# PolyChord/PolyChordLite

Hardware: AMD Instinct MI355X
Metric: likelihood evals/sec, 20D Gaussian nlive=2000 (higher is better)
Workload: dtype f64; 1 GPU; configs[1]: 20-D Gaussian, nlive=2000, num_repeats=40, one full run per step; batch_chains=1000, parallelism=repeat-sharded x1, mode=one run at a time per GPU; R runs in step: roofline.in_step

## Files before the change

include/polychord_hip.h:

```cpp
#ifndef POLYCHORD_HIP_H
#define POLYCHORD_HIP_H
#include <stdbool.h>
#ifdef __cplusplus
extern "C" {
#endif


typedef double (*polychord_loglike_fn)(double *theta, int nDims, double *phi, int nDerived);
typedef void (*polychord_prior_fn)(double *cube, double *theta, int nDims);
typedef void (*polychord_dumper_fn)(int ndead, int nlive, int npars, double *live, double *dead,
                                    double *logweights, double logZ, double logZerr);

void polychord_c_interface(
    polychord_loglike_fn loglikelihood, polychord_prior_fn prior, polychord_dumper_fn dumper,
    int nlive, int num_repeats, int nprior, int nfail, bool do_clustering, int feedback,
    double precision_criterion, double logzero, int max_ndead, double boost_posterior,
    bool posteriors, bool equals, bool cluster_posteriors, bool write_resume, bool write_paramnames,
    bool read_resume, bool write_stats, bool write_live, bool write_dead, bool write_prior,
    bool maximise, double compression_factor, bool synchronous, int nDims, int nDerived,
    char *base_dir, char *file_root, int nGrade, double *grade_frac, int *grade_dims, int n_nlives,
    double *loglikes, int *nlives, int seed, int *comm);

void polychord_c_interface_ini(polychord_loglike_fn loglikelihood, void (*setup_loglikelihood)(void),
                               char *inifile, int *comm);
// ... 246 lines not shown
                        unsigned batch, int nchains, const double *seeds, const double *chol,
                        double contour, double *babies_out, double *nhats_out, int *nlike_out);
#define PCHIP_NO_SUCH_PATH 64
int  pchip_directions(const pchip_settings *s, const pchip_like *like, const pchip_prior *prior, unsigned batch, int nchains,
                      const double *seeds, const double *chol, int path, double *nhat_out, double *nhat_w_out,
                      double *nhat_Ms_out, double *ch_My_out, int *has_Ms, double *raw_out, int nrows, int nbases);
int  pchip_prior_transform(const pchip_prior *prior, int nDims, int n, const double *cube, double *theta, int device);
int  pchip_update_factors(const pchip_settings *s, int ncluster, int nlive, const double *live, const int *live_cluster,
                          int nph, const double *phantom, const double *ph_logL, const int *ph_cluster, const double *threshold,
                          const double *shift, int path, double *cov, double *chol, int *count, double *shift_out, int *chol_suspect);
typedef struct {
    int ncluster, nlive, nph;
    const double *live, *live_logL; const int *live_cluster;
    const double *phantom, *ph_logL; const int *ph_cluster;
} pchip_cluster_in;
typedef struct {
    int maxc, nsplit_cap, scratch_cap;
    int ncluster, nsplit, levels, scratch_n;
    int *live_cluster, *live_pos, *cl_list;
    int *cl_n, *imin_slot, *ph_count; unsigned *cl_uid;
    double *logLp, *lse_ref, *lse_sum, *logXp, *logZp, *logZXp, *logZp2, *logZpXp;
    double *XpXq;
    int *ph_cluster;
    unsigned *split_child, *split_parent; double *split_logfrac;
    double *init;
    double *scratch_Sm; int *scratch_knn, *scratch_lab;
} pchip_cluster_out;
int  pchip_cluster_update(const pchip_settings *s, int nsets, const pchip_cluster_in *in, pchip_cluster_out *out, int path);

int  pchip_park_pack(int nchains, int nDims, const int *need, const double *prop, int *rank, int *count, double *cube, int device);
int  pchip_park_pack_many(int nruns, const int *nchains, int nDims, const int *need, const double *prop, int *rank, int *counts, int *total,
                          double *cube, int device);

#ifdef __cplusplus
}
#endif
#endif
```

polychordlite_amd/_ctypes_api.py:

```python
import ctypes as C
import os

import numpy as np

_HERE = os.path.dirname(os.path.abspath(__file__))
LIB_PATH = os.environ.get("PCHIP_LIB") or os.path.join(_HERE, "libpolychord_hip.so")

LOGLIKE_FN = C.CFUNCTYPE(C.c_double, C.POINTER(C.c_double), C.c_int, C.POINTER(C.c_double), C.c_int)
PRIOR_FN = C.CFUNCTYPE(None, C.POINTER(C.c_double), C.POINTER(C.c_double), C.c_int)
DUMPER_FN = C.CFUNCTYPE(None, C.c_int, C.c_int, C.c_int, C.POINTER(C.c_double), C.POINTER(C.c_double),
                        C.POINTER(C.c_double), C.c_double, C.c_double)

LIKE_CALLBACK, LIKE_GAUSSIAN, LIKE_RASTRIGIN, LIKE_TWIN_GAUSSIAN, LIKE_CORR_GAUSSIAN, LIKE_SOURCE = range(6)
KERNEL_CLASSES = ("k_nhats", "k_slice", "k_consume", "k_apply", "k_clean", "k_covmats", "k_bases_side")
LIKE_KINDS = {"gaussian": LIKE_GAUSSIAN, "rastrigin": LIKE_RASTRIGIN, "twin_gaussian": LIKE_TWIN_GAUSSIAN,
              "corr_gaussian": LIKE_CORR_GAUSSIAN, "source": LIKE_SOURCE}


class Settings(C.Structure):
    _fields_ = [("nDims", C.c_int), ("nDerived", C.c_int), ("nlive", C.c_int), ("num_repeats", C.c_int),
                ("nprior", C.c_int), ("nfail", C.c_int), ("do_clustering", C.c_int),
                ("precision_criterion", C.c_double), ("logzero", C.c_double), ("max_ndead", C.c_int),
                ("boost_posterior", C.c_double), ("posteriors", C.c_int), ("equals", C.c_int),
                ("cluster_posteriors", C.c_int), ("compression_factor", C.c_double), ("n_nlives", C.c_int),
# ... 91 lines not shown
    pr = np.ascontiguousarray(prop, dtype=np.float64)
    out = np.zeros_like(pr) if cube is None else cube
    assert out.flags.c_contiguous and out.dtype == np.float64 and out.shape == pr.shape
    rank = np.empty(nd.size, dtype=np.int32)
    cnt = C.c_int(-1)
    ip = C.POINTER(C.c_int)
    lib.pchip_park_pack.argtypes = [C.c_int, C.c_int, ip, C.POINTER(C.c_double), ip, ip, C.POINTER(C.c_double), C.c_int]
    lib.pchip_park_pack.restype = C.c_int
    rc = lib.pchip_park_pack(pr.shape[0], pr.shape[1], nd.ctypes.data_as(ip), dptr(pr), rank.ctypes.data_as(ip), C.byref(cnt), dptr(out), device)
    if rc:
        raise RuntimeError(f"pchip_park_pack failed with code {rc}")
    return rank, cnt.value, out


def park_pack_many(nchains, need, prop, cube=None, device=-1):
    lib = load()
    nc = np.ascontiguousarray(nchains, dtype=np.int32)
    nd = np.ascontiguousarray(need, dtype=np.int32)
    pr = np.ascontiguousarray(prop, dtype=np.float64)
    out = np.zeros_like(pr) if cube is None else cube
    assert out.flags.c_contiguous and out.dtype == np.float64 and out.shape == pr.shape
    assert nc.ndim == 1 and pr.ndim == 2 and nd.size == pr.shape[0] == int(nc.sum())
    rank = np.empty(nd.size, dtype=np.int32)
    counts = np.full(nc.size, -1, dtype=np.int32)
    tot = C.c_int(-1)
    ip = C.POINTER(C.c_int)
    lib.pchip_park_pack_many.argtypes = [C.c_int, ip, C.c_int, ip, C.POINTER(C.c_double), ip, ip, ip, C.POINTER(C.c_double), C.c_int]
    lib.pchip_park_pack_many.restype = C.c_int
    rc = lib.pchip_park_pack_many(nc.size, nc.ctypes.data_as(ip), pr.shape[1], nd.ctypes.data_as(ip), dptr(pr), rank.ctypes.data_as(ip),
                                  counts.ctypes.data_as(ip), C.byref(tot), dptr(out), device)
    if rc:
        raise RuntimeError(f"pchip_park_pack_many failed with code {rc}")
    return rank, counts, tot.value, out


_lib = None


def load():
    global _lib
    if _lib is not None:
        return _lib
    if not os.path.exists(LIB_PATH):
        raise ImportError(f"{LIB_PATH} is missing: build it with `python -m polychordlite_amd.build` "
                          "(hipcc --offload-arch=gfx950).  There is no CPU fallback.")
    lib = C.CDLL(LIB_PATH, mode=C.RTLD_GLOBAL)
    lib.pchip_settings_default.argtypes = [C.POINTER(Settings), C.c_int, C.c_int]
    lib.pchip_settings_default.restype = None
    lib.pchip_device_count.restype = C.c_int
    lib.pchip_run.argtypes = [C.POINTER(Settings), C.POINTER(Like), C.POINTER(Prior), C.POINTER(Result)]
    lib.pchip_run.restype = C.c_int
    lib.pchip_result_free.argtypes = [C.POINTER(Result)]
    lib.pchip_result_free.restype = None
    lib.pchip_slice_chains.argtypes = [C.POINTER(Settings), C.POINTER(Like), C.POINTER(Prior), C.c_uint, C.c_int,
                                       C.POINTER(C.c_double), C.POINTER(C.c_double), C.c_double,
                                       C.POINTER(C.c_double), C.POINTER(C.c_double), C.POINTER(C.c_int)]
    lib.pchip_slice_chains.restype = C.c_int
    lib.pchip_directions.argtypes = [C.POINTER(Settings), C.POINTER(Like), C.POINTER(Prior), C.c_uint, C.c_int, C.POINTER(C.c_double),
                                     C.POINTER(C.c_double), C.c_int, C.POINTER(C.c_double), C.POINTER(C.c_double), C.POINTER(C.c_double),
                                     C.POINTER(C.c_double), C.POINTER(C.c_int), C.POINTER(C.c_double), C.c_int, C.c_int]
    lib.pchip_directions.restype = C.c_int
    lib.polychord_hip_set_gaussian.argtypes = [C.c_double, C.c_double]
    lib.polychord_hip_set_uniform_prior.argtypes = [C.c_int, C.POINTER(C.c_double), C.POINTER(C.c_double)]
    lib.polychord_hip_set_corr_gaussian.argtypes = [C.c_int, C.POINTER(C.c_double), C.POINTER(C.c_double), C.c_double]
    lib.polychord_hip_set_option.argtypes = [C.c_char_p, C.c_double]
    lib.polychord_hip_set_sub_clustering.argtypes = [C.c_int, C.POINTER(C.c_int)]
# ... 475 lines not shown
```

polychordlite_amd/csrc/pc_engine.hip:

```cpp
#include "pc_state.h"
#include "pc_resume.h"
#include "pc_prior_table.h"
#include "pc_launch.h"
#include "pc_plan.h"
#include <cstdio>
#include <cstdlib>
#include <cstring>
#include <cstdarg>
#include <cstdint>
#include <new>
#include <cmath>
#include <vector>
#include <memory>
#include <string>
#include <chrono>
#include <algorithm>
#include <map>
#include <unordered_map>
#include <atomic>
#include <mutex>
#include <thread>
#include <functional>
#include <exception>
#include <ucontext.h>
// ... 2252 lines not shown
}

int pchip_park_pack(int nchains, int nDims, const int *need, const double *prop, int *rank, int *count, double *cube, int device)
{
    if (nchains < 1 || nDims < 1 || !need || !prop || !rank || !count || !cube) { pc_abi_set_last_error("pchip_park_pack: nchains >= 1 flags and rows of nDims >= 1, and room for the ranks, the count and the rows"); return 1; }
    int ndev = 0;
    if (hipGetDeviceCount(&ndev) != hipSuccess || ndev == 0) { (void)hipGetLastError(); std::fprintf(stderr, "polychord_hip: no HIP device available -- this engine has no CPU path\n"); return 2; }
    if (hipSetDevice(device >= 0 ? device % ndev : 0) != hipSuccess) return 2;
    const size_t nb = sizeof(double) * (size_t)nchains * nDims, ni = sizeof(int) * (size_t)nchains;
    int *d_need = nullptr, *d_rank = nullptr, *d_count = nullptr, *h_count = nullptr; double *d_prop = nullptr, *d_cube = nullptr;
    int rc = 2;
    if (hipMalloc(&d_need, ni) == hipSuccess && hipMalloc(&d_rank, ni) == hipSuccess && hipMalloc(&d_count, sizeof(int)) == hipSuccess &&
        hipMalloc(&d_prop, nb) == hipSuccess && hipMalloc(&d_cube, nb) == hipSuccess && hipHostMalloc(&h_count, sizeof(int)) == hipSuccess &&
        hipMemcpy(d_need, need, ni, hipMemcpyHostToDevice) == hipSuccess && hipMemcpy(d_prop, prop, nb, hipMemcpyHostToDevice) == hipSuccess &&
        hipMemcpy(d_cube, cube, nb, hipMemcpyHostToDevice) == hipSuccess) {
        void *dp = nullptr;
        *h_count = -1;
        if (hipHostGetDevicePointer(&dp, h_count, 0) == hipSuccess) {
            pc_launch_park_pack(nchains, nDims, d_need, 1, d_prop, d_rank, d_count, (int *)dp, d_cube, nullptr);
            int dc = -2;
            if (hipDeviceSynchronize() == hipSuccess && hipMemcpy(rank, d_rank, ni, hipMemcpyDeviceToHost) == hipSuccess &&
                hipMemcpy(&dc, d_count, sizeof(int), hipMemcpyDeviceToHost) == hipSuccess && hipMemcpy(cube, d_cube, nb, hipMemcpyDeviceToHost) == hipSuccess) {
                *count = *(volatile int *)h_count;
                rc = dc == *count ? 0 : 2;
            }
        }
    }
    if (rc) (void)hipGetLastError();
    (void)hipFree(d_need); (void)hipFree(d_rank); (void)hipFree(d_count); (void)hipFree(d_prop); (void)hipFree(d_cube);
    if (h_count) (void)hipHostFree(h_count);
    return rc;
}

int pchip_park_pack_many(int nruns, const int *nchains, int nDims, const int *need, const double *prop, int *rank, int *counts, int *total,
                         double *cube, int device)
{
    if (nruns < 1 || nruns > PC_PARK_MAX_RUNS || nDims < 1 || !nchains || !need || !prop || !rank || !counts || !total || !cube) {
        pc_abi_set_last_error("pchip_park_pack_many: 1 <= nruns <= 64 runs of nchains[r] >= 1 flags and rows of nDims >= 1, and room for the ranks, the counts, the total and the rows");
        return 1;
    }
    size_t all = 0; int max_chains = 0;
    for (int r = 0; r < nruns; ++r) {
        if (nchains[r] < 1) { pc_abi_set_last_error("pchip_park_pack_many: every run has at least one chain"); return 1; }
        all += (size_t)nchains[r]; max_chains = std::max(max_chains, nchains[r]);
    }
    int ndev = 0;
    if (hipGetDeviceCount(&ndev) != hipSuccess || ndev == 0) { (void)hipGetLastError(); std::fprintf(stderr, "polychord_hip: no HIP device available -- this engine has no CPU path\n"); return 2; }
    if (hipSetDevice(device >= 0 ? device % ndev : 0) != hipSuccess) return 2;
    const size_t nb = sizeof(double) * all * nDims, ni = sizeof(int) * all;
    int *d_need = nullptr, *d_rank = nullptr, *d_count = nullptr, *h_count = nullptr; double *d_prop = nullptr, *d_cube = nullptr; PcParkRun *h_runs = nullptr;
    int rc = 2;
    if (hipMalloc(&d_need, ni) == hipSuccess && hipMalloc(&d_rank, ni) == hipSuccess && hipMalloc(&d_count, sizeof(int) * PC_PARK_MAX_RUNS) == hipSuccess &&
        hipMalloc(&d_prop, nb) == hipSuccess && hipMalloc(&d_cube, nb) == hipSuccess && hipHostMalloc(&h_count, sizeof(int) * (PC_PARK_MAX_RUNS + 1)) == hipSuccess &&
        hipHostMalloc(&h_runs, sizeof(PcParkRun) * PC_PARK_MAX_RUNS) == hipSuccess &&
        hipMemcpy(d_need, need, ni, hipMemcpyHostToDevice) == hipSuccess && hipMemcpy(d_prop, prop, nb, hipMemcpyHostToDevice) == hipSuccess &&
        hipMemcpy(d_cube, cube, nb, hipMemcpyHostToDevice) == hipSuccess) {
        size_t o = 0;
        for (int r = 0; r < nruns; ++r) { h_runs[r] = PcParkRun{d_need + o, d_prop + o * nDims, d_rank + o, nchains[r], 1}; o += (size_t)nchains[r]; }
        for (int r = 0; r <= nruns; ++r) h_count[r] = -1;
        void *dp = nullptr, *dr = nullptr;
        if (hipHostGetDevicePointer(&dp, h_count, 0) == hipSuccess && hipHostGetDevicePointer(&dr, h_runs, 0) == hipSuccess &&
            pc_launch_park_pack_many(nruns, (const PcParkRun *)dr, max_chains, nDims, d_count, (int *)dp, d_cube, nullptr) == 0) {
            std::vector<int> dc((size_t)nruns, -2);
            if (hipDeviceSynchronize() == hipSuccess && hipMemcpy(rank, d_rank, ni, hipMemcpyDeviceToHost) == hipSuccess &&
                hipMemcpy(dc.data(), d_count, sizeof(int) * nruns, hipMemcpyDeviceToHost) == hipSuccess && hipMemcpy(cube, d_cube, nb, hipMemcpyDeviceToHost) == hipSuccess) {
                long sum = 0; rc = 0;
// ... 498 lines not shown
```

polychordlite_amd/csrc/pc_launch.h:

```cpp
#pragma once
#include "pc_state.h"
#include "../../include/polychord_hip.h"
#include <cstddef>
#include <memory>
#include <vector>

struct PcSourceForm {
    long nterms;
    int nsums;
    long nquad;
    long nshared;
    int has_prior;
    long long ndata, ntail;
    int alive;
};

static inline size_t pc_quad_lds(const PcSourceForm &f) { return f.nquad > 0 ? sizeof(double) * 2 * (size_t)((f.nquad + 1) & ~1L) : 0; }

static inline size_t pc_front_lds(const PcSourceForm &f) { return pc_quad_lds(f) + (f.nshared > 0 ? sizeof(double) * 2 * (size_t)((f.nshared + 1) & ~1L) : 0); }

static inline int pc_slice_phi_lds(const PcState *S, const PcSourceForm &f)
{
    const size_t sh0 = sizeof(double) * ((size_t)S->D + S->nr) + 16, tb = sizeof(double) * (size_t)S->nr * (S->D + 1);
    const size_t sums = sizeof(double) * (size_t)S->nr * (size_t)f.nsums;
// ... 40 lines not shown
int pc_launch_clean_many(const PcManyRec *dR, int R, int nblk_max, hipStream_t st);
void pc_launch_install_live(const PcState *S, const double *rows, int n, hipStream_t st);
void pc_launch_clean(const PcState *S, int nph, unsigned char *keep, int *blk, int *d_total, double *ph2, double *phL2, unsigned *phC2, unsigned long long *phU2, int *dst_index, hipStream_t st);
void pc_launch_reset_thresholds(const PcState *S, hipStream_t st);
int pc_launch_reset_thresholds_many(const PcState *S, const PcManyRec *dR, int R, hipStream_t st);
int pc_cov_nchunk(const PcState *S, int nph);
int pc_launch_covmats(const PcState *S, int nph, int nc, double *psum, int *pcnt, double *mean, int *count, double *pcov, hipStream_t st);
void pc_launch_scan_blocks(int *blk, int nblk, int *total, int *total2, hipStream_t st);
void pc_launch_chol_only(const PcState *S, const double *ncov, const int *count, hipStream_t st);
void pc_launch_init_state(const PcState *S, double logzero, hipStream_t st);
int pc_post_blocks(void);
void pc_launch_post_moments(const PcState *S, int nd, double *pmax, double *part, hipStream_t st);
void pc_prepare_streams(int dev, int want);
void *pc_cache_dev_alloc(size_t bytes);
void pc_cache_dev_free(void *p);
void *pc_cache_host_alloc(size_t bytes);
void pc_cache_host_free(void *p);
int pc_run_many(const pchip_settings *s, const pchip_like *like, const pchip_prior *prior, int nseeds, const int *seeds, int device, int max_in_flight, pchip_result *results);
void *pc_source_batch_open(int handle, int device, int nDims, int nDerived, polychord_prior_fn prior);
void pc_source_batch_eval(void *user, int n, int nDims, int nDerived, const double *cube, double *theta, double *phi, double *logL);
void pc_source_batch_close(void *user);
void pc_batch_callback_get(polychord_batch_fn *fn, void **user);
int pc_device_batch_registered(void);
int pc_fast_fits(const PcState *S);
int pc_launch_sort_live(const PcState *S, hipStream_t st);
int pc_launch_sort_live_many(const PcState *S, const PcManyRec *dR, int R, hipStream_t st);
int pc_launch_consume_fast(const PcState *S, int final_mode, hipStream_t st);
void pc_launch_ph_prepare(const PcState *S, hipStream_t st);
size_t pc_records_block_bytes(long long cap, int nT);
int pc_pack_lived_device(const double *dead, const double *logw, const double *entry, long long nd, int nT, double logzero, double *block, long long cap, long long *h_count, hipStream_t st);
int pc_par_fits(const PcState *S);
int pc_launch_consume_par(const PcState *S, hipStream_t st);
int pc_launch_consume_par_many(const PcState *S, const PcManyRec *dR, int R, hipStream_t st);
int pc_launch_final_par(const PcState *S, hipStream_t st);
int pc_launch_final_par_split(const PcState *S, hipStream_t st);
int pc_launch_final_par_many(const PcManyRec *dR, int R, hipStream_t st);
int pc_rtc_launch(const PcState *S, const char *expr, dim3 grid, dim3 block, size_t sh, hipStream_t st, void **args);
const char *pc_rtc_error(void);
int pc_rtc_source_form(int id, PcSourceForm *f);
int pc_rtc_wanted(const PcState *S);
int pc_launch_generate_live(const PcState *S, int attempt0, int n, double *rows, double *rows_logL, hipStream_t st);
int pc_nhats_splittable(const PcState *S);
int pc_launch_nhats_part(const PcState *S, unsigned batch, int nchains, int part, hipStream_t st, int packed);
int pc_launch_nhats(const PcState *S, unsigned batch, int nchains, hipStream_t st);
int pc_slice_fusable(const PcState *S);
int pc_launch_slice_fused(const PcState *S, unsigned batch, int nchains, hipStream_t st);
int pc_launch_slice_many(const PcState *S, const PcManyRec *dR, int R, int nchains, int fused, hipStream_t st);
int pc_launch_slice_step(const PcState *S, const PcManyRec *dR, int R, int nchains, int fused, hipStream_t st);
int pc_launch_nhats_many(const PcState *S, const PcManyRec *dR, int R, int nchains, hipStream_t st);
int pc_launch_slice(const PcState *S, unsigned batch, int nchains, hipStream_t st);
int pc_launch_prior_transform(const PcState *S, int n, const double *cubes, double *thetas, hipStream_t st);
int pc_launch_source_eval(const PcState *S, int n, const double *thetas, double *logL, double *phi, hipStream_t st);
int pc_launch_source_prior_eval(const PcState *S, int n, const double *cubes, double *thetas, hipStream_t st);
int pc_launch_max_rank(const PcState *S, int n, const double *rows, double *val, hipStream_t st);
int pc_launch_maximise(const PcState *S, int nprob, const double *in, const int *hdr, long long max_iter, double *out, long long *outi, hipStream_t st);
int pc_max_choose_simplex(int nDims, int nTotal, double logzero, const double *live, const int *cluster, int nlive, const double *vals,
                          double *simplex, double *f);
void pc_maximum_alloc(pchip_maximum *m, int nDims, int nDerived);
int pc_bases_t_ok(const PcState *S);
int pc_launch_bases_t(const PcState *S, unsigned batch, int nchains, hipStream_t st);
int pc_launch_bases_t_many(const PcState *S, const PcManyRec *dR, int R, unsigned batch, int nchains, hipStream_t st);
int pc_slice_t_ok(const PcState *S, int ncluster);
int pc_launch_slice_t(const PcState *S, unsigned batch, int nchains, hipStream_t st);
int pc_launch_slice_t_many(const PcState *S, const PcManyRec *dR, int R, unsigned batch, int nchains, hipStream_t st);
int pc_update_fused_ok(const PcState *S, int nc);
int pc_update_fused_blocks(const PcState *S, int nph);
// ... 13 lines not shown
```

polychordlite_amd/csrc/pc_par.hip:

```cpp
#include "pc_state.h"
#include "pc_launch.h"
#include "pc_keys.h"

typedef unsigned long long u64;
#define PAR_NT 1024
#define PAR_W 16

__device__ __forceinline__ int prefix_bits(const u64 *words, int t)
{
    int c = 0;
    const int wq = t >> 6;
    #pragma unroll
    for (int x = 0; x < PAR_W; ++x) {
        u64 v = words[x];
        if (x > wq) v = 0ull; else if (x == wq) v &= (1ull << (t & 63)) - 1ull;
        c += __popcll(v);
    }
    return c;
}

__device__ __forceinline__ int prefix_cum(const u64 *words, const int *cum, int t)
{
    const int wq = t >> 6;
    return (wq >= PAR_W) ? cum[PAR_W] : cum[wq] + __popcll(words[wq] & ((1ull << (t & 63)) - 1ull));
// ... 129 lines not shown
        R[q] = ref[q];
        const bool has = s[q] != 0.0 && m[q] > 0.5 * NEGBIG;
        const double d = m[q] - R[q];
        bad = bad || (has && !(fabs(d) <= PAR_LIN_SPAN));
        inc[q] = wave_scan_f64(has ? s[q] * exp(d) : 0.0, lane);
        if (lane == 63) sc[q * PAR_W + wv] = inc[q];
    }
    if (__ballot(bad) != 0ull && lane == 0) ref[NSEQ] = 1.0;
    pc_lds_barrier();
    const bool ok = ref[NSEQ] == 0.0;
    if (ok) {
        #pragma unroll
        for (int q = 0; q < NSEQ; ++q) {
            const double t = sc[q * PAR_W + (lane & 15)];
            double pre = t;
            pre += dpp_f64<0x111>(pre); pre += dpp_f64<0x112>(pre); pre += dpp_f64<0x114>(pre); pre += dpp_f64<0x118>(pre);
            s[q] = inc[q] + readlane_f64(pre - t, wv);
            m[q] = R[q];
        }
    }
    pc_lds_barrier();
    return ok;
}

__device__ __forceinline__ double block_scan_add(double v, int lane, int wv, double *wtot)
{
    v = wave_scan_f64(v, lane);
    if (lane == 63) wtot[wv] = v;
    __syncthreads();
    double p = 0.0;
    for (int x = 0; x < wv; ++x) p += wtot[x];
    __syncthreads();
    return v + p;
}

__device__ __forceinline__ void consume_par_body(const PcState &S)
{
    extern __shared__ __attribute__((aligned(16))) char smem[];
    const int tid = threadIdx.x, lane = tid & 63, wv = tid >> 6;
    const int Ncap = S.Ncap, nr = S.nr, NS = (Ncap + 63) & ~63;
    const int Bh = S.B;
    double bl = 0.0; int ep = 0, nl = 0;
    if (tid < Bh) { const int wh = Bh - 1 - tid; bl = S.baby_logL_T[(size_t)(nr - 1) * Bh + wh]; ep = S.ch_epoch[wh]; nl = S.ch_nlike[wh]; }
    PcCtl *ctl = S.ctl;
    const int T = ctl->i_nursery;
    const int n = S.cl_n[0];
    u64 *sSortK = (u64 *)smem;
    u64 *cK = sSortK + NS;
    u64 *srtK = cK + PAR_NT;
    u64 *uKey = srtK + PAR_NT;
    u64 *Gm = uKey + PAR_NT + 64;
    u64 *accR = Gm + PAR_NT;
    u64 *amask = accR + PAR_W;
    u64 *vmask = amask + PAR_W;
    double *sZi = (double *)(vmask + PAR_W);
    double *wtot = sZi + PAR_NT;
    double *fin = wtot + 64;
    int *sSort = (int *)(fin + 16);
    int *srtT = sSort + NS;
    int *rnk = srtT + PAR_NT;
    int *rlo = rnk + PAR_NT;
    int *uSrc = rlo + PAR_NT;
    int *slotA = uSrc + PAR_NT + 64;
    int *parA = slotA + PAR_NT;
    int *accStep = parA + PAR_NT;
    int *ish = accStep + PAR_NT;
    int *hist = ish + 16;
    double *X5 = (double *)(hist + NS + 64);
    double *sLse = (double *)Gm;

    const int epoch = ctl->admin_epoch;
    const int ndead0 = ctl->ndead, fail0 = ctl->failures, nph0 = ctl->nphantom;
    const long long nlike0 = ctl->nlike, niter0 = ctl->niter;
    const double logZ0 = ctl->logZ, logZ20 = ctl->logZ2;
    const double Xp0 = S.logXp[0], Zp0 = S.logZp[0], ZXp0 = S.logZXp[0], Zp20 = S.logZp2[0], ZpXp0 = S.logZpXp[0], XX0 = S.XpXq[0];
    const double lseRef0 = S.lse_ref[0], lseSum0 = S.lse_sum[0];
    const unsigned cuid = S.cl_uid[0];
    const double log2v = 0.6931471805599453;
    __shared__ int cumA[PAR_W + 1], cumV[PAR_W + 1], cumR[PAR_W + 1];
    __shared__ double ulog[4];
    if (wv == PAR_W - 1 && lane < 4) ulog[lane] = log(lane == 3 ? lseSum0 : (double)n + (double)lane);

    long long cyc[9]; int ncy = 0;
    cyc[ncy++] = clock64();
    for (int s = tid; s < Ncap; s += PAR_NT) { S.slot_src[s] = -1; if (S.defer_update) S.slot_step[s] = -1; }
    for (int i = tid; i < NS; i += PAR_NT) { sSortK[i] = (i < n) ? S.sort_key[i] : KEY_HUGE; sSort[i] = S.sort_slot[i]; }
    const bool inT = tid < T;
    const int w = T - 1 - tid;
    u64 ck = KEY_HUGE; bool valid = false;
    if (T != Bh && inT) { bl = S.baby_logL_T[(size_t)(nr - 1) * S.B + w]; ep = S.ch_epoch[w]; nl = S.ch_nlike[w]; }
    if (inT) { ck = d2key(bl); valid = ep == epoch; } else nl = 0;
    cK[tid] = ck;
    for (int i = tid; i < NS + 64; i += PAR_NT) hist[i] = 0;
    {
        const u64 vm = __ballot(valid);
        if (lane == 0) { vmask[wv] = vm; accR[wv] = 0ull; amask[wv] = 0ull; }
    }
    if (tid == 0) { ish[0] = (T << 2) | 3; ish[1] = 0; ish[3] = 0; }
    __syncthreads();
    const double l0 = ulog[0], l1 = ulog[1], l2 = ulog[2], d01 = l0 - l1, d02 = l0 - l2;

    int rl = 0, rp = 0;
    if (inT) {
        int lo = 0, hi = n;
        while (lo < hi) { const int mid = (lo + hi) >> 1; if (sSortK[mid] < ck) lo = mid + 1; else hi = mid; }
        rl = lo; rp = lo;
        while (rp < n && sSortK[rp] == ck) rp++;
    }
    rlo[tid] = rl;

    cyc[ncy++] = clock64();
    int myoff = 0;
    if (inT) myoff = atomicAdd(&hist[rl], 1);
    __syncthreads();
    {
        const int nb = n + 2;
        const int per = (nb + PAR_NT - 1) / PAR_NT, b0 = tid * per;
        int sum = 0;
        for (int x = 0; x < per; ++x) if (b0 + x < nb) sum += hist[b0 + x];
        int inc = sum;
        inc = wave_scan_i32(inc, lane);
        if (lane == 63) accStep[wv] = inc;
        __syncthreads();
        int run = inc - sum;
        for (int x = 0; x < wv; ++x) run += accStep[x];
        for (int x = 0; x < per; ++x) if (b0 + x < nb) { const int cnt = hist[b0 + x]; hist[b0 + x] = run; run += cnt; }
    }
    __syncthreads();
    if (inT) srtT[hist[rl] + myoff] = tid;
    __syncthreads();
    int rho = tid;
    if (inT) {
        const int g0 = hist[rl], g1 = hist[rl + 1];
        int below = 0;
        for (int x = g0; x < g1; ++x) {
            const int o = srtT[x];
            const u64 ko = cK[o];
            below += (ko < ck) || (ko == ck && o > tid);
        }
        rho = g0 + below;
    }
    rnk[tid] = rho;

    cyc[ncy++] = clock64();
    {
        u64 G = 0ull;
        #pragma unroll
        for (int j = 0; j < 64; ++j) {
            const int rj = __builtin_amdgcn_readlane(rho, j);
            if (j < lane && rj > rho) G |= 1ull << j;
        }
        Gm[tid] = G;
    }
    __syncthreads();
    if (wv == 0) {
        const int nch = (T + 63) >> 6;
        int *cum = accStep;
        if (lane < PAR_W) cum[lane] = 0;
        __threadfence_block();
        int rho_t = rnk[lane], r = rlo[lane], tot = 0;
        u64 Gt = Gm[lane];
        for (int c = 0; c < nch; ++c) {
            const int tn = (c + 1 < nch) ? (c + 1) * 64 + lane : lane;
            const int nrho = rnk[tn], nr2 = rlo[tn];
            const u64 nG = Gm[tn];
            const bool v = (vmask[c] >> lane) & 1ull;
            const int wq = rho_t >> 6, bq = rho_t & 63;
            const int P = tot - cum[wq] - __popcll(accR[wq] & (((1ull << bq) << 1) - 1ull));
            u64 am = __ballot(v && r > P);
            for (int it = 0; it < 66; ++it) {
                const bool a = v && r > P + __popcll(Gt & am);
                const u64 nm = __ballot(a);
                if (nm == am) break;
                am = nm;
            }
            if ((am >> lane) & 1ull) atomicOr(&accR[wq], 1ull << bq);
            if (lane == 0) amask[c] = am;
            tot += __popcll(am);
            PAR_WAVE_ORDER();
            {
                int cw = (lane < PAR_W) ? __popcll(accR[lane]) : 0, inc = cw;
                inc += dpp_i32<0x111>(inc); inc += dpp_i32<0x112>(inc); inc += dpp_i32<0x114>(inc); inc += dpp_i32<0x118>(inc);
                if (lane < PAR_W) cum[lane] = inc - cw;
            }
            PAR_WAVE_ORDER();
            rho_t = nrho; r = nr2; Gt = nG;
        }
        {
            const int ca = (lane < PAR_W) ? __popcll(amask[lane]) : 0, cv = (lane < PAR_W) ? __popcll(vmask[lane]) : 0,
                      cr = (lane < PAR_W) ? __popcll(accR[lane]) : 0;
            int ia = ca, iv = cv, ir = cr;
            ia += dpp_i32<0x111>(ia); ia += dpp_i32<0x112>(ia); ia += dpp_i32<0x114>(ia); ia += dpp_i32<0x118>(ia);
            iv += dpp_i32<0x111>(iv); iv += dpp_i32<0x112>(iv); iv += dpp_i32<0x114>(iv); iv += dpp_i32<0x118>(iv);
            ir += dpp_i32<0x111>(ir); ir += dpp_i32<0x112>(ir); ir += dpp_i32<0x114>(ir); ir += dpp_i32<0x118>(ir);
            if (lane < PAR_W) { cumA[lane] = ia - ca; cumV[lane] = iv - cv; cumR[lane] = ir - cr; }
            if (lane == PAR_W - 1) { cumA[PAR_W] = ia; cumV[PAR_W] = iv; cumR[PAR_W] = ir; }
        }
    }
    __syncthreads();

    cyc[ncy++] = clock64();
    const u64 amw = amask[wv], ltm = (1ull << lane) - 1ull;
    const bool acc = (amw >> lane) & 1ull;
    const int kt = cumA[wv] + __popcll(amw & ltm);
    const int K = cumA[PAR_W];
    const int vp = cumV[wv] + __popcll(vmask[wv] & ltm);
    int pos = 0, q = 0;
    if (acc) {
        q = cumR[rho >> 6] + __popcll(accR[rho >> 6] & ((1ull << (rho & 63)) - 1ull));
        pos = q + rp;
        accStep[kt] = tid; srtK[q] = ck;
    }
    __syncthreads();
    const u64 *aK = srtK;

    for (int idx = tid; idx <= K && idx < n; idx += PAR_NT) {
        const u64 sk = sSortK[idx];
        int lo = 0, hi = K;
        while (lo < hi) { const int mid = (lo + hi) >> 1; if (aK[mid] < sk) lo = mid + 1; else hi = mid; }
        const int p2 = idx + lo;
        if (p2 <= K) { uKey[p2] = sk; uSrc[p2] = sSort[idx]; }
    }
    if (acc && pos <= K) { uKey[pos] = ck; uSrc[pos] = -(1 + tid); }
    __syncthreads();

    const u64 gk = inT ? uKey[kt] : KEY_HUGE;
    const int src = acc ? uSrc[kt] : 0;
    slotA[tid] = (acc && src >= 0) ? src : -1;
    parA[tid] = (acc && src < 0) ? (-src - 1) : -1;
    __syncthreads();
    for (int it = 0; it < 12; ++it) {
        const int p = parA[tid];
// ... 254 lines not shown
            if (x > (ts >> 6)) word = 0ull; else if (x == (ts >> 6)) word &= (1ull << (ts & 63)) - 1ull;
            if (word) { tl = x * 64 + 63 - __clzll((long long)word); break; }
        }
        ctl->failures = (tl >= 0) ? vps - prefix_cum(vmask, cumV, tl) - 1 : fail0 + vps;
        ctl->status = status; ctl->error = (pri == 2) ? PC_ERR_DEAD_CAP : PC_ERR_NONE;
        ctl->i_nursery = T - ts; ctl->ndead = ndead0 + vps; ctl->seg_hi = T - 1; ctl->seg_lo = T - ts; ctl->cluster_deleted = 0;
        ctl->nlike = nlike0 + ish[1]; ctl->niter = niter0 + ts; ctl->nphantom = ish[2]; ctl->nlike_failed += ish[3];
        if (Kp) { ctl->logZ = fin[0]; ctl->logZ2 = fin[4]; }
        if (pri == 0) ctl->logX_last_update = Xp;
        ctl->upd_pending = 0; ctl->upd_marks = 0;
        if (marks_sh[1] > 0) {
            const int Kl = marks_sh[0], marks = marks_sh[1];
            ctl->upd_pending = 1; ctl->upd_marks = marks;
            ctl->upd_tmark = accStep[Kl - 1] + 1; ctl->upd_T = T; ctl->upd_ts = ts; ctl->upd_nph0 = S.pool ? S.pool_base : nph0;
            ctl->upd_thr = key2d(uKey[Kl - 1]); ctl->upd_keep_thr = (Kp > Kl) ? 1 : 0;
            ctl->logX_last_update = Xp0 + (double)Kl * d01;
        }
        if (S.use_prec) ctl->live_logZ = (Kp ? sLse[Kp - 1] : lseRef0 + ulog[3]) - l0 + Xp;
        cyc[ncy++] = clock64();
#ifdef PAR_NO_DBG
#elif defined(PAR_DBG_EVID)
        for (int x = 0; x < 7; ++x) ctl->dbg[x] += ecy[x + 1] - ecy[x];
#elif defined(PAR_DBG_PUBLISH)
        pcy[6] = clock64();
        for (int x = 0; x < 6; ++x) ctl->dbg[x] += pcy[x + 1] - pcy[x];
#else
        for (int x = 0; x + 1 < ncy && x < 8; ++x) ctl->dbg[x] += cyc[x + 1] - cyc[x];
        ctl->dbg[7] += npair;
#endif
    }
}
__global__ __launch_bounds__(PAR_NT) void k_consume_par(PcState S) { consume_par_body(S); }
__global__ __launch_bounds__(PAR_NT) void k_consume_par_many(const PcManyRec *R) { consume_par_body(pc_many_state(R, blockIdx.y)); }


template <bool ROWS>
__device__ __forceinline__ void final_par_body(const PcState &S)
{
    __shared__ __attribute__((aligned(16))) double X0[PAR_NT], X1[PAR_NT], X2[PAR_NT], X3[PAR_NT];
    __shared__ double wtot[64];
    __shared__ double carry[12];
    const int tid = threadIdx.x, lane = tid & 63, wv = tid >> 6;
    PcCtl *ctl = S.ctl;
    const int n0 = S.cl_n[0], nT = S.nT, ndead0 = ctl->ndead;
    const unsigned cuid = S.cl_uid[0];
    const double log2v = 0.6931471805599453;
    if (ndead0 + n0 > S.Dcap) { if (tid == 0) { ctl->status = PC_ST_ERROR; ctl->error = PC_ERR_DEAD_CAP; } return; }
    if (tid == 0) {
        carry[0] = ctl->logZ; carry[1] = ctl->logZ2; carry[2] = S.logXp[0]; carry[3] = S.XpXq[0]; carry[4] = S.logZp[0];
        carry[5] = S.logZXp[0]; carry[6] = S.logZp2[0]; carry[7] = S.logZpXp[0]; carry[8] = S.death_thr[0];
    }
    __syncthreads();
    for (int base = 0; base < n0; base += PAR_NT) {
        const int m = min(PAR_NT, n0 - base), i = base + tid;
        const bool on = tid < m;
        const double logZ0 = carry[0], logZ20 = carry[1], Xp0 = carry[2], XX0 = carry[3], Zp0 = carry[4], ZXp0 = carry[5],
                     Zp20 = carry[6], ZpXp0 = carry[7];
        const int slot = on ? S.sort_slot[i] : 0;
        const double L = on ? key2d(S.sort_key[i]) : NEGBIG;
        const int myn = n0 - i;
        const double a0 = on ? log((double)myn) : 0.0, a1 = on ? log((double)myn + 1.0) : 0.0, a2 = on ? log((double)myn + 2.0) : 0.0;
        const double e01 = a0 - a1, e02 = a0 - a2;
        const double sx = block_scan_add(e01, lane, wv, wtot), sxx = block_scan_add(e02, lane, wv, wtot);
        const double Xb = Xp0 + (sx - e01), XXb = XX0 + (sxx - e02), Sd = sx;
        double tM = on ? Xb + L - a1 : NEGBIG, tS = on ? 1.0 : 0.0;
        double vM = on ? (XXb + L + a0 - a1 - a2) - Sd : NEGBIG, vS = tS;
// ... 109 lines not shown
```

polychordlite_amd/csrc/pc_state.h:

```cpp
#pragma once
#include "pc_dev.h"

enum { PC_ST_RUNNING = 0, PC_ST_DONE = 1, PC_ST_UPDATE = 2, PC_ST_ERROR = 4 };
enum { PC_ERR_NONE = 0, PC_ERR_PHANTOM_CAP = 1, PC_ERR_DEAD_CAP = 2, PC_ERR_CLUSTER_CAP = 3, PC_ERR_NOSLOT = 4 };

enum { PC_ABL_FUNCTOR = 1 << 0, PC_ABL_NO_POOL = 1 << 1, PC_ABL_NO_DEFER = 1 << 2, PC_ABL_NO_FUSED_UPDATE = 1 << 3, PC_ABL_PAIR_SCANS = 1 << 4,
       PC_ABL_CONSUME_GENERAL = 1 << 5, PC_ABL_SLICE_LANE = 1 << 6, PC_ABL_BASES_PACKED = 1 << 7, PC_ABL_CL_END_AT_DEATH = 1 << 8,
       PC_ABL_KILLOFF_GENERAL = 1 << 9, PC_ABL_CONSUME_CL_SERIAL = 1 << 10, PC_ABL_RETIRED_11 = 1 << 11, PC_ABL_RETIRED_12 = 1 << 12,
       PC_ABL_NO_HELPER = 1 << 13, PC_ABL_QC_BY_CHAIN = 1 << 14, PC_ABL_RTC_BUILTINS = 1 << 15, PC_ABL_UPDATE_CHAIN = 1 << 16, PC_ABL_FLAG_LAUNCH = 1 << 17,
       PC_ABL_TRACE_CHOL = 1 << 30 };

#define PC_MASK_WORDS 16

struct PcCtl {
    int status;
    int error;
    int i_nursery;
    int admin_epoch;
    int failures;
    int ncluster;
    int ncluster_dead;
    int ndead;
    int nphantom;
    int seg_hi, seg_lo;
    int cluster_deleted;
    unsigned batch_id;
    unsigned next_cluster_uid;
    long long nlike;
    long long niter;
    long long nlike_device;
    long long nlike_failed;
    double logZ, logZ2;
    double logX_last_update;
    double live_logZ;
    unsigned long long seq;
    long long dbg[8];
    long long gen_cyc[4];
    long long nn_walks, nn_fallbacks;
    int upd_pending, upd_marks;
    int upd_tmark;
    int upd_T, upd_ts;
    int upd_nph0;
    int upd_keep_thr;
// ... 217 lines not shown
```

Baseline: 1.356 billion likelihood evals/s.

## Replace serial wave-0 acceptance fixpoint with block-parallel bitmap prefix acceptance

The acceptance step in the consume kernel used to run in wave 0 alone, walking 64-candidate chunks in order and iterating a ballot fixpoint inside each chunk. It now computes, for every thread in parallel, how many earlier candidates rank above it. This uses per-wave and per-16-lane rank bitmaps with prefix popcounts, plus DPP row comparisons within each 16-lane group. The goal is to remove the serial chunk loop from the critical path, at the cost of extra LDS atomics and barriers. The old path stays available behind an ablation flag, and a standalone test entry point and kernel are added.

```diff
diff --git a/include/polychord_hip.h b/include/polychord_hip.h
--- a/include/polychord_hip.h
+++ b/include/polychord_hip.h
@@ -302,6 +302,9 @@
 int  pchip_park_pack_many(int nruns, const int *nchains, int nDims, const int *need, const double *prop, int *rank, int *counts, int *total,
                           double *cube, int device);
 
+int  pchip_par_accept(int n, const double *snapshot_logL, int T, const double *cand_logL, const unsigned char *valid, int serial,
+                      unsigned char *accept, int device);
+
 #ifdef __cplusplus
 }
 #endif
diff --git a/polychordlite_amd/_ctypes_api.py b/polychordlite_amd/_ctypes_api.py
--- a/polychordlite_amd/_ctypes_api.py
+++ b/polychordlite_amd/_ctypes_api.py
@@ -147,6 +147,23 @@
     if rc:
         raise RuntimeError(f"pchip_park_pack_many failed with code {rc}")
     return rank, counts, tot.value, out
+
+
+def par_accept(snapshot_logL, cand_logL, valid=None, serial=False, device=-1):
+    lib = load()
+    sn = np.ascontiguousarray(snapshot_logL, dtype=np.float64)
+    cd = np.ascontiguousarray(cand_logL, dtype=np.float64)
+    vl = np.ones(cd.size, dtype=np.uint8) if valid is None else np.ascontiguousarray(np.asarray(valid) != 0, dtype=np.uint8)
+    assert sn.ndim == 1 and cd.ndim == 1 and vl.shape == cd.shape
+    acc = np.full(cd.size, 0xEE, dtype=np.uint8)
+    bp = C.POINTER(C.c_ubyte)
+    lib.pchip_par_accept.argtypes = [C.c_int, C.POINTER(C.c_double), C.c_int, C.POINTER(C.c_double), bp, C.c_int, bp, C.c_int]
+    lib.pchip_par_accept.restype = C.c_int
+    rc = lib.pchip_par_accept(sn.size, dptr(sn), cd.size, dptr(cd), vl.ctypes.data_as(bp), 1 if serial else 0, acc.ctypes.data_as(bp), device)
+    if rc:
+        raise RuntimeError(f"pchip_par_accept failed with code {rc}")
+    assert np.all(acc <= 1)
+    return acc.astype(bool)
 
 
 _lib = None
diff --git a/polychordlite_amd/csrc/pc_engine.hip b/polychordlite_amd/csrc/pc_engine.hip
--- a/polychordlite_amd/csrc/pc_engine.hip
+++ b/polychordlite_amd/csrc/pc_engine.hip
@@ -2308,6 +2308,32 @@
     return rc;
 }
 
+int pchip_par_accept(int n, const double *snapshot_logL, int T, const double *cand_logL, const unsigned char *valid, int serial,
+                     unsigned char *accept, int device)
+{
+    if (n < 1 || n > 8192 || T < 1 || T > 1024 || !snapshot_logL || !cand_logL || !valid || !accept) {
+        pc_abi_set_last_error("pchip_par_accept: 1 <= n <= 8192 ascending snapshot values, 1 <= T <= 1024 candidates with their flags, and room for T answers");
+        return 1;
+    }
+    for (int i = 1; i < n; ++i) if (!(snapshot_logL[i - 1] <= snapshot_logL[i])) { pc_abi_set_last_error("pchip_par_accept: the snapshot is not ascending"); return 1; }
+    int ndev = 0;
+    if (hipGetDeviceCount(&ndev) != hipSuccess || ndev == 0) { (void)hipGetLastError(); std::fprintf(stderr, "polychord_hip: no HIP device available -- this engine has no CPU path\n"); return 2; }
+    if (hipSetDevice(device >= 0 ? device % ndev : 0) != hipSuccess) return 2;
+    double *d_snap = nullptr, *d_cand = nullptr; unsigned char *d_valid = nullptr, *d_acc = nullptr;
+    int rc = 2;
+    if (hipMalloc(&d_snap, sizeof(double) * (size_t)n) == hipSuccess && hipMalloc(&d_cand, sizeof(double) * (size_t)T) == hipSuccess &&
+        hipMalloc(&d_valid, (size_t)T) == hipSuccess && hipMalloc(&d_acc, (size_t)T) == hipSuccess &&
+        hipMemcpy(d_snap, snapshot_logL, sizeof(double) * (size_t)n, hipMemcpyHostToDevice) == hipSuccess &&
+        hipMemcpy(d_cand, cand_logL, sizeof(double) * (size_t)T, hipMemcpyHostToDevice) == hipSuccess &&
+        hipMemcpy(d_valid, valid, (size_t)T, hipMemcpyHostToDevice) == hipSuccess && hipMemset(d_acc, 0xEE, (size_t)T) == hipSuccess) {
+        if (pc_launch_par_accept(n, d_snap, T, d_cand, d_valid, serial, d_acc, nullptr) == 0 && hipDeviceSynchronize() == hipSuccess &&
+            hipMemcpy(accept, d_acc, (size_t)T, hipMemcpyDeviceToHost) == hipSuccess) rc = 0;
+    }
+    if (rc) (void)hipGetLastError();
+    (void)hipFree(d_snap); (void)hipFree(d_cand); (void)hipFree(d_valid); (void)hipFree(d_acc);
+    return rc;
+}
+
 int pchip_park_pack_many(int nruns, const int *nchains, int nDims, const int *need, const double *prop, int *rank, int *counts, int *total,
                          double *cube, int device)
 {
diff --git a/polychordlite_amd/csrc/pc_launch.h b/polychordlite_amd/csrc/pc_launch.h
--- a/polychordlite_amd/csrc/pc_launch.h
+++ b/polychordlite_amd/csrc/pc_launch.h
@@ -96,6 +96,8 @@
 int pc_par_fits(const PcState *S);
 int pc_launch_consume_par(const PcState *S, hipStream_t st);
 int pc_launch_consume_par_many(const PcState *S, const PcManyRec *dR, int R, hipStream_t st);
+int pc_launch_par_accept(int n, const double *snap, int T, const double *cand, const unsigned char *valid, int serial, unsigned char *accept,
+                         hipStream_t st);
 int pc_launch_final_par(const PcState *S, hipStream_t st);
 int pc_launch_final_par_split(const PcState *S, hipStream_t st);
 int pc_launch_final_par_many(const PcManyRec *dR, int R, hipStream_t st);
diff --git a/polychordlite_amd/csrc/pc_par.hip b/polychordlite_amd/csrc/pc_par.hip
--- a/polychordlite_amd/csrc/pc_par.hip
+++ b/polychordlite_amd/csrc/pc_par.hip
@@ -185,6 +185,176 @@
     for (int x = 0; x < wv; ++x) p += wtot[x];
     __syncthreads();
     return v + p;
+}
+
+struct ParAcc {
+    const u64 *sSortK;
+    const u64 *cK;
+    int *hist;
+    int *srtT;
+    int *accStep;
+    int *rnk, *rlo;
+    u64 *Gm;
+    u64 *accR, *amask;
+    const u64 *vmask;
+    u64 *cmap;
+    u64 *ccum;
+    int *ccnt;
+    u64 *smap;
+    u64 *scum;
+    int *scnt;
+    int *cumA, *cumV, *cumR;
+};
+
+__device__ __forceinline__ void par_search(const u64 *sSortK, int n, u64 ck, bool inT, int &rl, int &rp)
+{
+    if (inT) {
+        int lo = 0, hi = n;
+        while (lo < hi) { const int mid = (lo + hi) >> 1; if (sSortK[mid] < ck) lo = mid + 1; else hi = mid; }
+        rl = lo; rp = lo;
+        while (rp < n && sSortK[rp] == ck) rp++;
+    }
+}
+
+__device__ __forceinline__ int par_rank(const ParAcc &A, int n, u64 ck, bool inT, int rl, int tid, int lane, int wv)
+{
+    const u64 *cK = A.cK; int *hist = A.hist, *srtT = A.srtT, *accStep = A.accStep;
+    int myoff = 0;
+    if (inT) myoff = atomicAdd(&hist[rl], 1);
+    __syncthreads();
+    {
+        const int nb = n + 2;
+        const int per = (nb + PAR_NT - 1) / PAR_NT, b0 = tid * per;
+        int sum = 0;
+        for (int x = 0; x < per; ++x) if (b0 + x < nb) sum += hist[b0 + x];
+        int inc = sum;
+        inc = wave_scan_i32(inc, lane);
+        if (lane == 63) accStep[wv] = inc;
+        __syncthreads();
+        int run = inc - sum;
+        for (int x = 0; x < wv; ++x) run += accStep[x];
+        for (int x = 0; x < per; ++x) if (b0 + x < nb) { const int cnt = hist[b0 + x]; hist[b0 + x] = run; run += cnt; }
+    }
+    __syncthreads();
+    if (inT) srtT[hist[rl] + myoff] = tid;
+    __syncthreads();
+    int rho = tid;
+    if (inT) {
+        const int g0 = hist[rl], g1 = hist[rl + 1];
+        int below = 0;
+        for (int x = g0; x < g1; ++x) {
+            const int o = srtT[x];
+            const u64 ko = cK[o];
+            below += (ko < ck) || (ko == ck && o > tid);
+        }
+        rho = g0 + below;
+    }
+    return rho;
+}
+
+#define PAR_ROW_STEP(K) { const int o = __builtin_amdgcn_update_dpp(-1, rhoV, 0x110 + K, 0xF, 0xF, false); inrow += o > rho; }
+__device__ __forceinline__ void par_accept(const ParAcc &A, int T, bool serial, bool valid, int rl, int rho, int tid, int lane, int wv)
+{
+    int *rnk = A.rnk, *rlo = A.rlo, *accStep = A.accStep, *cumA = A.cumA, *cumV = A.cumV, *cumR = A.cumR;
+    u64 *Gm = A.Gm, *accR = A.accR, *amask = A.amask; const u64 *vmask = A.vmask;
+    int inrow = 0;
+    if (serial) {
+        u64 G = 0ull;
+        #pragma unroll
+        for (int j = 0; j < 64; ++j) {
+            const int rj = __builtin_amdgcn_readlane(rho, j);
+            if (j < lane && rj > rho) G |= 1ull << j;
+        }
+        Gm[tid] = G;
+    } else {
+        if (valid) {
+            atomicOr(&A.cmap[wv * PAR_W + (rho >> 6)], 1ull << (rho & 63));
+            atomicOr(&A.smap[(tid >> 4) * PAR_W + (rho >> 6)], 1ull << (rho & 63));
+        }
+        const int rhoV = valid ? rho : -1;
+        PAR_ROW_STEP(1) PAR_ROW_STEP(2) PAR_ROW_STEP(3) PAR_ROW_STEP(4) PAR_ROW_STEP(5) PAR_ROW_STEP(6) PAR_ROW_STEP(7) PAR_ROW_STEP(8)
+        PAR_ROW_STEP(9) PAR_ROW_STEP(10) PAR_ROW_STEP(11) PAR_ROW_STEP(12) PAR_ROW_STEP(13) PAR_ROW_STEP(14) PAR_ROW_STEP(15)
+    }
+    __syncthreads();
+    if (!serial) {
+        {
+            const int s = tid >> 4;
+            u64 o = 0ull;
+            for (int x = s & ~3; x < s; ++x) o |= A.smap[x * PAR_W + (tid & 15)];
+            A.scum[tid] = o;
+            const int cw = __popcll(o); int inc = cw;
+            inc += dpp_i32<0x111>(inc); inc += dpp_i32<0x112>(inc); inc += dpp_i32<0x114>(inc); inc += dpp_i32<0x118>(inc);
+            A.scnt[tid] = inc - cw;
+            if ((tid & 15) == PAR_W - 1) A.scnt[PAR_NT + s] = inc;
+        }
+        if (tid < PAR_W * PAR_W) {
+            const int c = tid >> 4;
+            u64 o = 0ull;
+            for (int x = 0; x < c; ++x) o |= A.cmap[x * PAR_W + (tid & 15)];
+            A.ccum[tid] = o;
+            const int cw = __popcll(o); int inc = cw;
+            inc += dpp_i32<0x111>(inc); inc += dpp_i32<0x112>(inc); inc += dpp_i32<0x114>(inc); inc += dpp_i32<0x118>(inc);
+            A.ccnt[tid] = inc - cw;
+            if ((tid & 15) == PAR_W - 1) A.ccnt[PAR_W * PAR_W + c] = inc;
+        }
+        __syncthreads();
+        const int wq = rho >> 6, bq = rho & 63, s = tid >> 4;
+        const u64 le = ((1ull << bq) << 1) - 1ull;
+        const int P = A.ccnt[PAR_W * PAR_W + wv] - A.ccnt[wv * PAR_W + wq] - __popcll(A.ccum[wv * PAR_W + wq] & le)
+                      + A.scnt[PAR_NT + s] - A.scnt[s * PAR_W + wq] - __popcll(A.scum[s * PAR_W + wq] & le) + inrow;
+        const bool a = valid && rl > P;
+        const u64 am = __ballot(a);
+        if (lane == 0) amask[wv] = am;
+        if (a) atomicOr(&accR[wq], 1ull << bq);
+        __syncthreads();
+    }
+    if (wv == 0) {
+        if (serial) {
+            const int nch = (T + 63) >> 6;
+            int *cum = accStep;
+            if (lane < PAR_W) cum[lane] = 0;
+            __threadfence_block();
+            int rho_t = rnk[lane], r = rlo[lane], tot = 0;
+            u64 Gt = Gm[lane];
+            for (int c = 0; c < nch; ++c) {
+                const int tn = (c + 1 < nch) ? (c + 1) * 64 + lane : lane;
+                const int nrho = rnk[tn], nr2 = rlo[tn];
+                const u64 nG = Gm[tn];
+                const bool v = (vmask[c] >> lane) & 1ull;
+                const int wq = rho_t >> 6, bq = rho_t & 63;
+                const int P = tot - cum[wq] - __popcll(accR[wq] & (((1ull << bq) << 1) - 1ull));
+                u64 am = __ballot(v && r > P);
+                for (int it = 0; it < 66; ++it) {
+                    const bool a = v && r > P + __popcll(Gt & am);
+                    const u64 nm = __ballot(a);
+                    if (nm == am) break;
+                    am = nm;
+                }
+                if ((am >> lane) & 1ull) atomicOr(&accR[wq], 1ull << bq);
+                if (lane == 0) amask[c] = am;
+                tot += __popcll(am);
+                PAR_WAVE_ORDER();
+                {
+                    int cw = (lane < PAR_W) ? __popcll(accR[lane]) : 0, inc = cw;
+                    inc += dpp_i32<0x111>(inc); inc += dpp_i32<0x112>(inc); inc += dpp_i32<0x114>(inc); inc += dpp_i32<0x118>(inc);
+                    if (lane < PAR_W) cum[lane] = inc - cw;
+                }
+                PAR_WAVE_ORDER();
+                rho_t = nrho; r = nr2; Gt = nG;
+            }
+        }
+        {
+            const int ca = (lane < PAR_W) ? __popcll(amask[lane]) : 0, cv = (lane < PAR_W) ? __popcll(vmask[lane]) : 0,
+                      cr = (lane < PAR_W) ? __popcll(accR[lane]) : 0;
+            int ia = ca, iv = cv, ir = cr;
+            ia += dpp_i32<0x111>(ia); ia += dpp_i32<0x112>(ia); ia += dpp_i32<0x114>(ia); ia += dpp_i32<0x118>(ia);
+            iv += dpp_i32<0x111>(iv); iv += dpp_i32<0x112>(iv); iv += dpp_i32<0x114>(iv); iv += dpp_i32<0x118>(iv);
+            ir += dpp_i32<0x111>(ir); ir += dpp_i32<0x112>(ir); ir += dpp_i32<0x114>(ir); ir += dpp_i32<0x118>(ir);
+            if (lane < PAR_W) { cumA[lane] = ia - ca; cumV[lane] = iv - cv; cumR[lane] = ir - cr; }
+            if (lane == PAR_W - 1) { cumA[PAR_W] = ia; cumV[PAR_W] = iv; cumR[PAR_W] = ir; }
+        }
+    }
+    __syncthreads();
 }
 
 __device__ __forceinline__ void consume_par_body(const PcState &S)
@@ -221,6 +391,8 @@
     int *hist = ish + 16;
     double *X5 = (double *)(hist + NS + 64);
     double *sLse = (double *)Gm;
+    u64 *cmap = uKey, *smap = srtK, *scum = (u64 *)sZi;
+    const bool acc_serial = (S.ablate & PC_ABL_ACCEPT_SERIAL) != 0;
 
     const int epoch = ctl->admin_epoch;
     const int ndead0 = ctl->ndead, fail0 = ctl->failures, nph0 = ctl->nphantom;
@@ -249,108 +421,23 @@
         const u64 vm = __ballot(valid);
         if (lane == 0) { vmask[wv] = vm; accR[wv] = 0ull; amask[wv] = 0ull; }
     }
+    if (tid < PAR_W * PAR_W) cmap[tid] = 0ull;
+    smap[tid] = 0ull;
     if (tid == 0) { ish[0] = (T << 2) | 3; ish[1] = 0; ish[3] = 0; }
     __syncthreads();
     const double l0 = ulog[0], l1 = ulog[1], l2 = ulog[2], d01 = l0 - l1, d02 = l0 - l2;
 
     int rl = 0, rp = 0;
-    if (inT) {
-        int lo = 0, hi = n;
-        while (lo < hi) { const int mid = (lo + hi) >> 1; if (sSortK[mid] < ck) lo = mid + 1; else hi = mid; }
-        rl = lo; rp = lo;
-        while (rp < n && sSortK[rp] == ck) rp++;
-    }
+    par_search(sSortK, n, ck, inT, rl, rp);
     rlo[tid] = rl;
 
     cyc[ncy++] = clock64();
-    int myoff = 0;
-    if (inT) myoff = atomicAdd(&hist[rl], 1);
-    __syncthreads();
-    {
-        const int nb = n + 2;
-        const int per = (nb + PAR_NT - 1) / PAR_NT, b0 = tid * per;
-        int sum = 0;
-        for (int x = 0; x < per; ++x) if (b0 + x < nb) sum += hist[b0 + x];
-        int inc = sum;
-        inc = wave_scan_i32(inc, lane);
-        if (lane == 63) accStep[wv] = inc;
-        __syncthreads();
-        int run = inc - sum;
-        for (int x = 0; x < wv; ++x) run += accStep[x];
-        for (int x = 0; x < per; ++x) if (b0 + x < nb) { const int cnt = hist[b0 + x]; hist[b0 + x] = run; run += cnt; }
-    }
-    __syncthreads();
-    if (inT) srtT[hist[rl] + myoff] = tid;
-    __syncthreads();
-    int rho = tid;
-    if (inT) {
-        const int g0 = hist[rl], g1 = hist[rl + 1];
-        int below = 0;
-        for (int x = g0; x < g1; ++x) {
-            const int o = srtT[x];
-            const u64 ko = cK[o];
-            below += (ko < ck) || (ko == ck && o > tid);
-        }
-        rho = g0 + below;
-    }
+    const ParAcc A = { sSortK, cK, hist, srtT, accStep, rnk, rlo, Gm, accR, amask, vmask, cmap, cmap + PAR_W * PAR_W, uSrc, smap, scum, slotA, cumA, cumV, cumR };
+    const int rho = par_rank(A, n, ck, inT, rl, tid, lane, wv);
     rnk[tid] = rho;
 
     cyc[ncy++] = clock64();
-    {
-        u64 G = 0ull;
-        #pragma unroll
-        for (int j = 0; j < 64; ++j) {
-            const int rj = __builtin_amdgcn_readlane(rho, j);
-            if (j < lane && rj > rho) G |= 1ull << j;
-        }
-        Gm[tid] = G;
-    }
-    __syncthreads();
-    if (wv == 0) {
-        const int nch = (T + 63) >> 6;
-        int *cum = accStep;
-        if (lane < PAR_W) cum[lane] = 0;
-        __threadfence_block();
-        int rho_t = rnk[lane], r = rlo[lane], tot = 0;
-        u64 Gt = Gm[lane];
-        for (int c = 0; c < nch; ++c) {
-            const int tn = (c + 1 < nch) ? (c + 1) * 64 + lane : lane;
-            const int nrho = rnk[tn], nr2 = rlo[tn];
-            const u64 nG = Gm[tn];
-            const bool v = (vmask[c] >> lane) & 1ull;
-            const int wq = rho_t >> 6, bq = rho_t & 63;
-            const int P = tot - cum[wq] - __popcll(accR[wq] & (((1ull << bq) << 1) - 1ull));
-            u64 am = __ballot(v && r > P);
-            for (int it = 0; it < 66; ++it) {
-                const bool a = v && r > P + __popcll(Gt & am);
-                const u64 nm = __ballot(a);
-                if (nm == am) break;
-                am = nm;
-            }
-            if ((am >> lane) & 1ull) atomicOr(&accR[wq], 1ull << bq);
-            if (lane == 0) amask[c] = am;
-            tot += __popcll(am);
-            PAR_WAVE_ORDER();
-            {
-                int cw = (lane < PAR_W) ? __popcll(accR[lane]) : 0, inc = cw;
-                inc += dpp_i32<0x111>(inc); inc += dpp_i32<0x112>(inc); inc += dpp_i32<0x114>(inc); inc += dpp_i32<0x118>(inc);
-                if (lane < PAR_W) cum[lane] = inc - cw;
-            }
-            PAR_WAVE_ORDER();
-            rho_t = nrho; r = nr2; Gt = nG;
-        }
-        {
-            const int ca = (lane < PAR_W) ? __popcll(amask[lane]) : 0, cv = (lane < PAR_W) ? __popcll(vmask[lane]) : 0,
-                      cr = (lane < PAR_W) ? __popcll(accR[lane]) : 0;
-            int ia = ca, iv = cv, ir = cr;
-            ia += dpp_i32<0x111>(ia); ia += dpp_i32<0x112>(ia); ia += dpp_i32<0x114>(ia); ia += dpp_i32<0x118>(ia);
-            iv += dpp_i32<0x111>(iv); iv += dpp_i32<0x112>(iv); iv += dpp_i32<0x114>(iv); iv += dpp_i32<0x118>(iv);
-            ir += dpp_i32<0x111>(ir); ir += dpp_i32<0x112>(ir); ir += dpp_i32<0x114>(ir); ir += dpp_i32<0x118>(ir);
-            if (lane < PAR_W) { cumA[lane] = ia - ca; cumV[lane] = iv - cv; cumR[lane] = ir - cr; }
-            if (lane == PAR_W - 1) { cumA[PAR_W] = ia; cumV[PAR_W] = iv; cumR[PAR_W] = ir; }
-        }
-    }
-    __syncthreads();
+    par_accept(A, T, acc_serial, valid, rl, rho, tid, lane, wv);
 
     cyc[ncy++] = clock64();
     const u64 amw = amask[wv], ltm = (1ull << lane) - 1ull;
@@ -671,6 +758,66 @@
 }
 __global__ __launch_bounds__(PAR_NT) void k_consume_par(PcState S) { consume_par_body(S); }
 __global__ __launch_bounds__(PAR_NT) void k_consume_par_many(const PcManyRec *R) { consume_par_body(pc_many_state(R, blockIdx.y)); }
+
+__global__ __launch_bounds__(PAR_NT) void k_par_accept(int n, const double *snap, int T, const double *cand, const unsigned char *valid_in,
+                                                       int serial, unsigned char *accept)
+{
+    extern __shared__ __attribute__((aligned(16))) char smem[];
+    const int tid = threadIdx.x, lane = tid & 63, wv = tid >> 6;
+    const int NS = (n + 63) & ~63;
+    u64 *sSortK = (u64 *)smem;
+    u64 *cK = sSortK + NS;
+    u64 *Gm = cK + PAR_NT;
+    u64 *cmap = Gm + PAR_NT;
+    u64 *smap = cmap + 2 * PAR_W * PAR_W;
+    u64 *accR = smap + 2 * PAR_NT;
+    u64 *amask = accR + PAR_W;
+    u64 *vmask = amask + PAR_W;
+    int *srtT = (int *)(vmask + PAR_W);
+    int *rnk = srtT + PAR_NT;
+    int *rlo = rnk + PAR_NT;
+    int *accStep = rlo + PAR_NT;
+    int *ccnt = accStep + PAR_NT;
+    int *scnt = ccnt + PAR_W * PAR_W + PAR_W;
+    int *hist = scnt + PAR_NT + 64;
+    __shared__ int cumA[PAR_W + 1], cumV[PAR_W + 1], cumR[PAR_W + 1];
+    for (int i = tid; i < NS; i += PAR_NT) sSortK[i] = (i < n) ? d2key(snap[i]) : KEY_HUGE;
+    const bool inT = tid < T;
+    u64 ck = KEY_HUGE; bool valid = false;
+    if (inT) { ck = d2key(cand[tid]); valid = valid_in[tid] != 0; }
+    cK[tid] = ck;
+    for (int i = tid; i < NS + 64; i += PAR_NT) hist[i] = 0;
+    {
+        const u64 vm = __ballot(valid);
+        if (lane == 0) { vmask[wv] = vm; accR[wv] = 0ull; amask[wv] = 0ull; }
+    }
+    if (tid < PAR_W * PAR_W) cmap[tid] = 0ull;
+    smap[tid] = 0ull;
+    __syncthreads();
+    int rl = 0, rp = 0;
+    par_search(sSortK, n, ck, inT, rl, rp);
+    rlo[tid] = rl;
+    const ParAcc A = { sSortK, cK, hist, srtT, accStep, rnk, rlo, Gm, accR, amask, vmask, cmap, cmap + PAR_W * PAR_W, ccnt, smap, smap + PAR_NT, scnt, cumA, cumV, cumR };
+    const int rho = par_rank(A, n, ck, inT, rl, tid, lane, wv);
+    rnk[tid] = rho;
+    par_accept(A, T, serial != 0, valid, rl, rho, tid, lane, wv);
+    if (inT) accept[tid] = (unsigned char)((amask[wv] >> lane) & 1ull);
+}
+#define PAR_DOOR_NMAX 8192
+static size_t par_door_lds(int n)
+{
+    const size_t NS = ((size_t)n + 63) & ~(size_t)63;
+    return 8 * (NS + 4 * PAR_NT + 2 * PAR_W * PAR_W + 3 * PAR_W) + 4 * (5 * PAR_NT + 64 + PAR_W * PAR_W + PAR_W + NS + 64);
+}
+extern "C" int pc_launch_par_accept(int n, const double *snap, int T, const double *cand, const unsigned char *valid, int serial,
+                                    unsigned char *accept, hipStream_t st)
+{
+    if (n < 1 || n > PAR_DOOR_NMAX || T < 1 || T > PAR_NT) return 1;
+    const size_t sh = par_door_lds(n);
+    pc_need_dyn_lds((const void *)k_par_accept, sh);
+    hipLaunchKernelGGL(k_par_accept, dim3(1), dim3(PAR_NT), sh, st, n, snap, T, cand, valid, serial, accept);
+    return 0;
+}
 
 
 template <bool ROWS>
diff --git a/polychordlite_amd/csrc/pc_state.h b/polychordlite_amd/csrc/pc_state.h
--- a/polychordlite_amd/csrc/pc_state.h
+++ b/polychordlite_amd/csrc/pc_state.h
@@ -8,7 +8,7 @@
        PC_ABL_CONSUME_GENERAL = 1 << 5, PC_ABL_SLICE_LANE = 1 << 6, PC_ABL_BASES_PACKED = 1 << 7, PC_ABL_CL_END_AT_DEATH = 1 << 8,
        PC_ABL_KILLOFF_GENERAL = 1 << 9, PC_ABL_CONSUME_CL_SERIAL = 1 << 10, PC_ABL_RETIRED_11 = 1 << 11, PC_ABL_RETIRED_12 = 1 << 12,
        PC_ABL_NO_HELPER = 1 << 13, PC_ABL_QC_BY_CHAIN = 1 << 14, PC_ABL_RTC_BUILTINS = 1 << 15, PC_ABL_UPDATE_CHAIN = 1 << 16, PC_ABL_FLAG_LAUNCH = 1 << 17,
-       PC_ABL_TRACE_CHOL = 1 << 30 };
+       PC_ABL_ACCEPT_SERIAL = 1 << 18, PC_ABL_TRACE_CHOL = 1 << 30 };
 
 #define PC_MASK_WORDS 16
 
```

Result: faster. 1.388 billion likelihood evals/s (median of 6 runs) (+2.4%).
